# perrysou/SoftGNSS-python

Measured on NVIDIA B200. Metric: tracking channel-ms/s, higher is better.
Workload: dtype int8 x Q38 fixed-point correlators (exact int32 dot products), f64 rotors / accumulation / loop filters

## Files before the change

### softgnss_python_b200/csrc/sgx_common.cuh

```cuda
#pragma once
#include <stdint.h>
#include <stdio.h>
#include <string.h>
#include <mutex>

#ifdef SGX_EMUL
#include "cuda_emul.h"
#else
#include <cuda_runtime.h>
#define SGX_LAUNCH(kernel, grid, block, smem, stream, ...) \
  kernel<<<(grid), (block), (smem), (stream)>>>(__VA_ARGS__)
#define SGX_DYN_SMEM(name) extern __shared__ __align__(1024) unsigned char name[]
#endif

#include "../../include/softgnss_b200.h"

#ifdef SGX_EMUL
#define SGX_TABLE static
#else
#define SGX_TABLE static __constant__
#endif

namespace sgx {

// ... 87 lines not shown
#ifndef SGX_EMUL
  asm volatile("cp.async.wait_all;\n" ::: "memory");
#endif
}

__device__ __forceinline__ void mbar_init(unsigned long long* bar, unsigned count) {
#ifdef SGX_EMUL
  *bar = 0;
  (void)count;
#else
  unsigned s = (unsigned)__cvta_generic_to_shared(bar);
  asm volatile("mbarrier.init.shared::cta.b64 [%0], %1;\n" ::"r"(s), "r"(count) : "memory");
  asm volatile("fence.mbarrier_init.release.cluster;\n" ::: "memory");
#endif
}
__device__ __forceinline__ unsigned smem_addr(const void* p) {
#ifdef SGX_EMUL
  (void)p; return 0u;
#else
  unsigned a = (unsigned)__cvta_generic_to_shared(p), o;
  asm volatile("mov.u32 %0, %1;" : "=r"(o) : "r"(a));
  return o;
#endif
}
__device__ __forceinline__ unsigned lds_u32(const void* base, unsigned base_s, int byte_off) {
#ifdef SGX_EMUL
  (void)base_s; return *reinterpret_cast<const unsigned*>(reinterpret_cast<const char*>(base) + byte_off);
#else
  (void)base; unsigned v;
  asm volatile("ld.shared.u32 %0, [%1];" : "=r"(v) : "r"(base_s + (unsigned)byte_off));
  return v;
#endif
}
__device__ __forceinline__ double2 lds_f64x2(const void* base, unsigned base_s, int byte_off) {
#ifdef SGX_EMUL
  (void)base_s; return *reinterpret_cast<const double2*>(reinterpret_cast<const char*>(base) + byte_off);
#else
  (void)base; double2 v;
  asm volatile("ld.shared.v2.f64 {%0, %1}, [%2];" : "=d"(v.x), "=d"(v.y) : "r"(base_s + (unsigned)byte_off));
  return v;
#endif
}

__device__ __forceinline__ void bulk_load(void* smem_dst, const void* gsrc, unsigned bytes,
                                          unsigned long long* bar) {
#ifdef SGX_EMUL
  memcpy(smem_dst, gsrc, bytes);
  *bar += 1;
#else
  unsigned d = (unsigned)__cvta_generic_to_shared(smem_dst);
  unsigned b = (unsigned)__cvta_generic_to_shared(bar);
  asm volatile("mbarrier.arrive.expect_tx.shared::cta.b64 _, [%0], %1;\n" ::"r"(b), "r"(bytes) : "memory");
  asm volatile(
      "cp.async.bulk.shared::cluster.global.mbarrier::complete_tx::bytes [%0], [%1], %2, [%3];\n" ::"r"(d),
      "l"(gsrc), "r"(bytes), "r"(b)
      : "memory");
#endif
}
__device__ __forceinline__ void mbar_wait(unsigned long long* bar, unsigned parity) {
#ifdef SGX_EMUL
  while ((*(volatile unsigned long long*)bar & 1ull) == (unsigned long long)parity) sgx_emul::yield_to_sched();
#else
  unsigned b = (unsigned)__cvta_generic_to_shared(bar);
  asm volatile(
      "{\n"
      ".reg .pred p;\n"
// ... 25 lines not shown
```

### softgnss_python_b200/csrc/sgx_track.cu

```cuda
#include <vector>
#include <fcntl.h>
#include <sys/stat.h>
#include <unistd.h>
#include "sgx_common.cuh"

namespace sgx {

constexpr int TRK_THREADS = 256;
constexpr int TRK_WARPS = TRK_THREADS / 32;
constexpr int TRK_MARGIN = 256;

struct TrackArgs {
  const int8_t* rec;
  long long rec_stride;
  const long long* rec_len;
  const sgx_channel* ch;
  const int8_t* chips;
  double* out;
  int* ms_done;
  int* status;
  int n_channels;
  int ms;
  int resume;
  long long avail;
  struct TrackState* state;
  long long* prof;
  int win;
  long long skip;
  long long abs_base;
  double fs, codeFreqBasis, codeLength, spc;
  double c1code, c2code, c1carr, c2carr;
};

struct MsParams {
  double startE, stepE, startL, stepL, startP, stepP;
  double inv_step;
  long long q0_fix, h_fix;
  double cps;
  double rem_cyc;
  double w;
  double rem_rad;
  double fs;
  long long pos;
// ... 43 lines not shown

__device__ __forceinline__ void cis_cycles(double cyc, float& c, float& s) {
  cyc -= rint(cyc);
  const float hi = (float)cyc;
  const float lo = (float)(cyc - (double)hi) * 6.2831853071795865f;
  float s0, c0;
  sincospif(2.0f * hi, &s0, &c0);
  c = fmaf(-s0, lo, c0);
  s = fmaf(c0, lo, s0);
}

__device__ __forceinline__ void cmul(float& r, float& i, float ar, float ai, float br, float bi) {
  r = fmaf(ar, br, -(ai * bi));
  i = fmaf(ar, bi, ai * br);
}

struct CodeState {
  double codeFreq, remCodePhase, oldCodeNco, oldCodeError, nextRemCode;
  long long pos;
};
struct CarrState {
  double carrFreq, carrFreqBasis, remCarrPhase, oldCarrNco, oldCarrError, w;
};

constexpr int SGX_PAUSED = 1;

struct TrackState {
  CodeState c;
  CarrState r;
  int k;
  int status;
};

__device__ void prepare_code(const TrackArgs& a, CodeState& st, long long rec_len, MsParams& p) {
  double step = st.codeFreq / a.fs;
  int blk = (int)ceil((a.codeLength - st.remCodePhase) / step);
  p.blk = blk;
  p.pos = st.pos;
  p.stop = 0;
  long long aligned = st.pos & ~15LL;
  if (st.pos + blk > rec_len) { p.stop = SGX_ERR_SHORT; return; }
  if (st.pos + blk > a.avail) { p.stop = SGX_PAUSED; return; }
  if (blk <= 0 || (st.pos - aligned) + blk > a.win) { p.stop = SGX_ERR_RANGE; return; }
  double rem = st.remCodePhase, spc = a.spc, bs = (double)blk * step;
  p.startE = rem - spc;
  p.stepE = (((bs + rem) - spc) - p.startE) / (double)blk;
  p.startL = rem + spc;
  p.stepL = (((bs + rem) + spc) - p.startL) / (double)blk;
  p.startP = rem;
  p.stepP = ((bs + rem) - p.startP) / (double)blk;
  p.inv_step = 1.0 / step;
  p.h_fix = __double2ll_rn(0.5 * p.inv_step * 1099511627776.0);
  p.q0_fix = __double2ll_rn(-rem * p.inv_step * 1099511627776.0);
  st.nextRemCode = (lin_y(blk - 1, p.stepP, p.startP) + step) - 1023.0;
}

__device__ void prepare_carr(const TrackArgs& a, CarrState& st, MsParams& p) {
  st.w = st.carrFreq * 2.0 * 3.141592653589793;
  p.cps = (st.w / a.fs) * 0.15915494309189535;
  p.rem_cyc = st.remCarrPhase * 0.15915494309189535;
  p.w = st.w;
  p.rem_rad = st.remCarrPhase;
  p.fs = a.fs;
}

__device__ double carry_carr_phase(const TrackArgs& a, const CarrState& st, int blk) {
  const double TWO_PI = 6.283185307179586;
  double arg_end = st.w * ((double)blk / a.fs) + st.remCarrPhase;
  double m;
  if (arg_end >= 0.0) {
    double q = floor(arg_end * 0.15915494309189535);
    m = __fma_rn(-q, TWO_PI, arg_end);
    if (m < 0.0) { q -= 1.0; m = __fma_rn(-q, TWO_PI, arg_end); }
    else if (m >= TWO_PI) { q += 1.0; m = __fma_rn(-q, TWO_PI, arg_end); }
  } else {
    m = fmod(arg_end, TWO_PI);
    if (m != 0.0 && m < 0.0) m += TWO_PI;
  }
  return m;
}

__device__ __forceinline__ void correlate_groups(const MsParams& P, const int8_t* cur, const float* codeS, int tid,
                                                 double& tEr, double& tEi, double& tPr, double& tPi, double& tLr,
                                                 double& tLi) {
    const int off = (int)(P.pos - (P.pos & ~15LL));
    const int ng = (off + P.blk + 15) >> 4;
    const int gpt = (ng + TRK_THREADS - 1) / TRK_THREADS;
    const int g0 = tid * gpt;
    const int g1 = min(g0 + gpt, ng);
    if (g0 < g1) {
      int ib = 16 * g0 - off;
      const int i0 = max(ib, 0);
      CodeVar E, Pm, L;
      E.init(i0, P.startE, P.stepE, P.inv_step, codeS);
      Pm.init(i0, P.startP, P.stepP, P.inv_step, codeS);
      L.init(i0, P.startL, P.stepL, P.inv_step, codeS);
      float wr[16], wi[16], w16r, w16i, rotr, roti;
      {
        cis_cycles((double)ib * P.cps + P.rem_cyc, rotr, roti);
        float s1, c1;
        cis_cycles(P.cps, c1, s1);
// ... 233 lines not shown
  const double r2 = r * r;
  double ps = -7.647163731819816e-13;
  ps = fma(ps, r2, 1.6059043836821613e-10);
  ps = fma(ps, r2, -2.505210838544172e-08);
  ps = fma(ps, r2, 2.7557319223985893e-06);
  ps = fma(ps, r2, -1.984126984126984e-04);
  ps = fma(ps, r2, 8.333333333333333e-03);
  ps = fma(ps, r2, -1.6666666666666666e-01);
  const double s0 = fma(ps * r2, r, r);
  double pc = 4.779477332387385e-14;
  pc = fma(pc, r2, -1.1470745597729725e-11);
  pc = fma(pc, r2, 2.08767569878681e-09);
  pc = fma(pc, r2, -2.755731922398589e-07);
  pc = fma(pc, r2, 2.48015873015873e-05);
  pc = fma(pc, r2, -1.388888888888889e-03);
  pc = fma(pc, r2, 4.1666666666666664e-02);
  pc = fma(pc, r2, -0.5);
  const double c0 = fma(pc, r2, 1.0);
  const int q = (int)(long long)k & 3;
  const double sa = (q & 1) ? c0 : s0, ca = (q & 1) ? s0 : c0;
  sn = (q & 2) ? -sa : sa;
  cs = ((q + 1) & 2) ? -ca : ca;
}

__device__ __forceinline__ void cis_cycles_f64(double cyc, double& c, double& s) {
  cyc -= rint(cyc);
  sincospi(2.0 * cyc, &s, &c);
}

template <int NW>
__device__ __forceinline__ void build_exact_tables(ExactTables& T, double cps, int lane) {
  constexpr int LMAX = 4 * NW;
  constexpr int ND = ExactDigits<NW>::value;
  if (lane < LMAX) {
    double c, s;
    cis_cycles_f64((double)lane * cps, c, s);
    const double one = (double)(1LL << (8 * ND - 2));
    long long w[2] = {__double2ll_rn(c * one), __double2ll_rn(s * one)};
#pragma unroll
    for (int q = 0; q < 2; ++q) {
      long long v = w[q];
#pragma unroll
      for (int d = 0; d < ND - 1; ++d) {
        const long long b = ((v + 128) & 0xFF) - 128;
        T.tw[q][d][lane] = (signed char)b;
        v = (v - b) >> 8;
      }
      T.tw[q][ND - 1][lane] = (signed char)v;
    }
  }
  constexpr int Z0 = (LMAX + 5 <= 32) ? LMAX : 0;
  if (lane >= Z0 && lane < Z0 + 5) {
    const int j = lane - Z0;
    cis_cycles_f64((double)(LMAX - 4 + j) * cps, T.z[j][0], T.z[j][1]);
  }
}

constexpr int IRREGULAR = 1 << 30;
__device__ __noinline__ int settle_boundary(int n, const MsParams& P) {
  if ((n & 1) == 0) return max(0, min(next_event(n >> 1, P.startP, P.stepP, P.inv_step), P.blk));
  const int c = (n - 1) >> 1;
  const int b = next_event(c, P.startE, P.stepE, P.inv_step);
  const int bl = next_event(c + 1, P.startL, P.stepL, P.inv_step);
  return max(0, min(b, P.blk)) | (bl != b ? IRREGULAR : 0);
}

__device__ __noinline__ double2 start_rotor(int a, const MsParams& P) {
  const double th = P.w * ((double)a / P.fs) + P.rem_rad;
  double sn, cs;
  if (fabs(th) < 5.0e5) sincos_reduced(th, sn, cs);
  else sincos(th, &sn, &cs);
  return make_double2(cs, sn);
}

__device__ __noinline__ void correlate_per_sample(const MsParams& P, const int8_t* cur, const unsigned char* codeB, int off,
                                                  int i0, int i1, double* acc) {
  for (int i = i0; i < i1; ++i) {
    const int ie = (int)ceil(lin_y(i, P.stepE, P.startE));
    const int ip = (int)ceil(lin_y(i, P.stepP, P.startP));
    const int il = (int)ceil(lin_y(i, P.stepL, P.startL));
    double cs, sn;
    cis_cycles_f64((double)i * P.cps + P.rem_cyc, cs, sn);
    const double x = (double)cur[off + i];
    const double pr = x * cs, pi = x * sn;
    const double ce = codeB[ie] ? -1.0 : 1.0, cp = codeB[ip] ? -1.0 : 1.0, cl = codeB[il] ? -1.0 : 1.0;
    acc[0] += ce * pr; acc[1] += ce * pi;
    acc[2] += cp * pr; acc[3] += cp * pi;
    acc[4] += cl * pr; acc[5] += cl * pi;
// ... 2 lines not shown

__device__ __forceinline__ double flip_sign(double x, unsigned m) {
  return __hiloint2double(__double2hiint(x) ^ (int)m, __double2loint(x));
}

__device__ __forceinline__ double digits_to_double(int lo, int mid, int hi) {
  long long v = (long long)mid * 65536 + (long long)lo;
  v += (long long)hi << 32;
  v += 0x4338000000000000LL;
  return __longlong_as_double(v) - 6755399441055744.0;
}

template <int NW, int SEGS>
__device__ __forceinline__ void correlate_exact(const MsParams& P, const MsParams& Pcold, const int8_t* cur,
                                                const unsigned char* codeB, const ExactTables& T, int tid,
                                                double& tEr, double& tEi, double& tPr, double& tPi, double& tLr,
                                                double& tLi) {
  constexpr int LMAX = 4 * NW;
  constexpr int ND = ExactDigits<NW>::value;
  static_assert(SEGS == 8, "sign bytes are fetched for 8 half-chip segments per thread");
  const int off = (int)(P.pos - (P.pos & ~15LL));
  const int n0 = SEGS * tid - 1;
  const long long FR_ONE = 1LL << 40, FR_EPS = 1099512;
  long long qf = P.q0_fix + (long long)n0 * P.h_fix;
  auto boundary = [&](int n, long long q) -> int {
    if (n < 0) return 0;
    if (n > 2046) return P.blk;
    const long long fr = q & (FR_ONE - 1);
    if (fr < FR_EPS || fr > FR_ONE - FR_EPS) return settle_boundary(n, Pcold);
    return max(0, min((int)(q >> 40) + 1, P.blk));
  };
  int a = boundary(n0, qf);
  if ((a & ~IRREGULAR) >= P.blk) return;
  int twr[ND][NW], twi[ND][NW];
#pragma unroll
  for (int d = 0; d < ND; ++d)
#pragma unroll
    for (int q = 0; q < NW; ++q) {
      twr[d][q] = reinterpret_cast<const int*>(T.tw[0][d])[q];
      twi[d][q] = reinterpret_cast<const int*>(T.tw[1][d])[q];
    }
  unsigned sg_lo = reinterpret_cast<const unsigned*>(codeB)[tid];
  unsigned sg_hi = reinterpret_cast<const unsigned*>(codeB)[tid + 1];
  double rotr = 1.0, roti = 0.0;
  double aEr = 0, aEi = 0, aPr = 0, aPi = 0, aLr = 0, aLi = 0;
  bool fresh = true;
  const unsigned cur_s = smem_addr(cur), z_s = smem_addr(&T.z[0][0]);
#pragma unroll 1
  for (int s = 0; s < SEGS; ++s) {
    qf += P.h_fix;
    const int b = boundary(n0 + s + 1, qf);
    const int len = (b & ~IRREGULAR) - (a & ~IRREGULAR);
    if (len > 0) {
      if (len > LMAX || ((a | b) & IRREGULAR)) {
        double acc[6] = {0, 0, 0, 0, 0, 0};
        correlate_per_sample(Pcold, cur, codeB, off, a & ~IRREGULAR, b & ~IRREGULAR, acc);
        const double up = (double)(1LL << (8 * ND - 2));
        aEr += acc[0] * up; aEi += acc[1] * up; aPr += acc[2] * up; aPi += acc[3] * up; aLr += acc[4] * up; aLi += acc[5] * up;
        fresh = true;
      } else {
        const unsigned mE = sg_lo << 24, mL = __byte_perm(sg_lo, 0u, 0x1444), mP = (s & 1) ? mL : mE;
        if (fresh) {
          const double2 r0 = start_rotor(a, Pcold);
          rotr = r0.x; roti = r0.y;
          fresh = false;
        }
        const int sh = ((off + a) & 3) * 8;
        unsigned raw[NW + 1];
        {
          const int wo = (off + a) & ~3;
#pragma unroll
          for (int q = 0; q <= NW; ++q) raw[q] = lds_u32(cur, cur_s, wo + 4 * q);
        }
        unsigned w[NW];
#pragma unroll
        for (int q = 0; q < NW; ++q) w[q] = __funnelshift_r(raw[q], raw[q + 1], sh);
        w[NW - 1] &= __funnelshift_lc(0xFFFFFFFFu, 0u, max(8 * (len - 4 * (NW - 1)), 0));
        if (len < LMAX - 4) {
#pragma unroll
          for (int q = 0; q < NW - 1; ++q) w[q] &= __funnelshift_lc(0xFFFFFFFFu, 0u, max(8 * (len - 4 * q), 0));
        }
        int xr[ND], xi[ND];
#pragma unroll
        for (int d = 0; d < ND; ++d) { xr[d] = 0; xi[d] = 0; }
#pragma unroll
        for (int q = 0; q < NW; ++q) {
#pragma unroll
          for (int d = 0; d < ND; ++d) {
            xr[d] = __dp4a((int)w[q], twr[d][q], xr[d]);
            xi[d] = __dp4a((int)w[q], twi[d][q], xi[d]);
          }
        }
        const double Sr = digits_to_double(xr[1] * 256 + xr[0], xr[3] * 256 + xr[2], ND == 5 ? xr[ND - 1] : 0);
        const double Si = digits_to_double(xi[1] * 256 + xi[0], xi[3] * 256 + xi[2], ND == 5 ? xi[ND - 1] : 0);
        const double Rr = fma(rotr, Sr, -(roti * Si)), Ri = fma(rotr, Si, roti * Sr);
        aEr += flip_sign(Rr, mE); aEi += flip_sign(Ri, mE);
        aPr += flip_sign(Rr, mP); aPi += flip_sign(Ri, mP);
        aLr += flip_sign(Rr, mL); aLi += flip_sign(Ri, mL);
        const int j = len - (LMAX - 4);
        if (j >= 0) {
          const double2 z = lds_f64x2(&T.z[0][0], z_s, 16 * j);
          const double zr = z.x, zi = z.y;
          const double nr = fma(rotr, zr, -(roti * zi)), ni = fma(rotr, zi, roti * zr);
          rotr = nr; roti = ni;
        } else {
          fresh = true;
        }
      }
    }
    a = b;
    if (s & 1) { sg_lo = __funnelshift_r(sg_lo, sg_hi, 8); sg_hi >>= 8; }
  }
  const double sc = 1.0 / (double)(1LL << (8 * ND - 2));
  tEr += aEr * sc; tEi += aEi * sc; tPr += aPr * sc; tPi += aPi * sc; tLr += aLr * sc; tLi += aLi * sc;
}

template <bool BULK, int NW, bool EXACT, int NT>
__global__ void __launch_bounds__(NT, 2) track_kernel(TrackArgs a) {
  SGX_DYN_SMEM(smem);
  int8_t* buf0 = (int8_t*)smem;
  int8_t* buf1 = buf0 + a.win;
  __shared__ MsParams prm;
  constexpr int NWARPS = NT / 32;
  __shared__ double red[NWARPS][6];
  __shared__ float codeS[1040];
  __shared__ unsigned long long mbar[2];
  __shared__ ExactTables xt;
  __shared__ CodeState cstS;
  __shared__ CarrState rstS;
  __shared__ __align__(4) unsigned char codeB[EXACT ? 1040 : 4];

  const int tid = threadIdx.x;
  const int cid = blockIdx.x;
  const int rid = cid / a.n_channels;
  const sgx_channel chn = a.ch[cid];
  if (chn.prn == 0) {
    if (tid == 0) {
      a.ms_done[cid] = 0;
      a.status[cid] = SGX_OK;
      if (a.state) { a.state[cid].k = 0; a.state[cid].status = SGX_OK; }
    }
    return;
  }
  const int8_t* rec = a.rec + (long long)rid * a.rec_stride;
  const long long rec_len = a.rec_len[rid];
  const long long rec_alloc = (rec_len + 15) & ~15LL;
  {
    const int8_t* c = a.chips + (chn.prn - 1) * 1023;
    for (int i = tid; i < 1040; i += NT) {
      codeS[i] = i < 1025 ? (float)c[(i + 1022) % 1023] : 0.f;
      if (EXACT) codeB[i] = codeS[i] < 0.f ? 0x80 : 0;
    }
  }
  int k_start = 0;
  if (a.resume) {
    const TrackState* ts = a.state + cid;
    if (ts->status != SGX_PAUSED) return;
    k_start = ts->k;
    if (tid == 0) { CodeState c = ts->c; prepare_code(a, c, rec_len, prm); cstS = c; }
    if (tid == 32) { CarrState r = ts->r; prepare_carr(a, r, prm); rstS = r; }
    if (tid == 0 && BULK) { mbar_init(&mbar[0], 1); mbar_init(&mbar[1], 1); }
  } else {
    if (tid == 0) {
      CodeState c;
      c.codeFreq = a.codeFreqBasis;
      c.remCodePhase = 0.0;
      c.oldCodeNco = c.oldCodeError = 0.0;
      c.nextRemCode = 0.0;
      c.pos = a.skip + (long long)chn.codePhase;
      prepare_code(a, c, rec_len, prm);
      cstS = c;
      if (BULK) { mbar_init(&mbar[0], 1); mbar_init(&mbar[1], 1); }
    }
    if (tid == 32) {
      CarrState r;
      r.carrFreq = chn.acquiredFreq;
      r.carrFreqBasis = chn.acquiredFreq;
      r.remCarrPhase = 0.0;
      r.oldCarrNco = r.oldCarrError = 0.0;
      prepare_carr(a, r, prm);
      rstS = r;
    }
  }
  if (EXACT && (tid >> 5) == 1) {
    const double cps = __shfl_sync(0xffffffffu, tid == 32 ? prm.cps : 0.0, 0);
    build_exact_tables<(NW > 0 ? NW : 1)>(xt, cps, tid & 31);
  }
  __syncthreads();

  auto stage = [&](int8_t* dst, long long pos) {
    long long al = pos & ~15LL;
    long long nb = rec_alloc - al;
    if (nb > a.win) nb = a.win;
    if (nb <= 0) return 0;
    if (BULK) {
      return (int)nb;
    } else {
      const int8_t* src = rec + al;
      for (int o = tid * 16; o < (int)nb; o += NT * 16) cp_async16(dst + o, src + o);
      cp_async_commit();
      return (int)nb;
    }
  };
  unsigned phase0 = 0, phase1 = 0;
  bool pending0 = false, pending1 = false;
  if (prm.stop == 0) {
    const int par = k_start & 1;
    int nb = stage(par ? buf1 : buf0, prm.pos);
    if (BULK) {
      if (nb > 0) {
        if (tid == 0) bulk_load(par ? buf1 : buf0, rec + (prm.pos & ~15LL), (unsigned)nb, &mbar[par]);
        if (par) pending1 = true; else pending0 = true;
      }
    }
  }

  int k = k_start;
  for (; k < a.ms; ++k) {
    const MsParams P = prm;
    if (P.stop != 0) break;
    long long t0 = 0, t1 = 0, t2 = 0, t3 = 0;
    if (a.prof && (tid == 0 || tid == 64)) t0 = clock64();
    int8_t* cur = (k & 1) ? buf1 : buf0;
    int8_t* nxt = (k & 1) ? buf0 : buf1;
    if (BULK) {
      if (k & 1) { if (pending1) { mbar_wait(&mbar[1], phase1); phase1 ^= 1; pending1 = false; } }
      else       { if (pending0) { mbar_wait(&mbar[0], phase0); phase0 ^= 1; pending0 = false; } }
    } else {
      if (k == k_start) { cp_async_wait_all(); __syncthreads(); }
    }
    {
      long long npos = P.pos + P.blk;
      int nb = stage(nxt, npos);
      if (BULK && nb > 0) {
        if (tid == 0) bulk_load(nxt, rec + (npos & ~15LL), (unsigned)nb, &mbar[(k + 1) & 1]);
        if (k & 1) pending0 = true; else pending1 = true;
      }
    }

    double tEr = 0.0, tEi = 0.0, tPr = 0.0, tPi = 0.0, tLr = 0.0, tLi = 0.0;
    if (EXACT)       correlate_exact<(NW > 0 ? NW : 1), 2048 / NT>(P, prm, cur, codeB, xt, tid, tEr, tEi, tPr, tPi, tLr, tLi);
    else if (NW > 0) correlate_segments<(NW > 0 ? NW : 1)>(P, cur, codeS, tid, tEr, tEi, tPr, tPi, tLr, tLi);
    else             correlate_groups(P, cur, codeS, tid, tEr, tEi, tPr, tPi, tLr, tLi);
    if (a.prof && (tid == 0 || tid == 64)) t1 = clock64();
    double v0 = warp_sum_f64(tEi), v1 = warp_sum_f64(tEr), v2 = warp_sum_f64(tPi), v3 = warp_sum_f64(tPr),
           v4 = warp_sum_f64(tLi), v5 = warp_sum_f64(tLr);
    if ((tid & 31) == 0) {
      double* r = red[tid >> 5];
      r[0] = v0; r[1] = v1; r[2] = v2; r[3] = v3; r[4] = v4; r[5] = v5;
    }
    if (!BULK) cp_async_wait_all();
    __syncthreads();
    if (a.prof && (tid == 0 || tid == 64)) t2 = clock64();
    if (tid == 0) {
      CodeState cst = cstS;
      double I_E = 0.0, Q_E = 0.0, I_L = 0.0, Q_L = 0.0;
      for (int w = 0; w < NWARPS; ++w) { I_E += red[w][0]; Q_E += red[w][1]; I_L += red[w][4]; Q_L += red[w][5]; }
      cst.remCodePhase = cst.nextRemCode;
      cst.pos = P.pos + P.blk;
      double em = sqrt(I_E * I_E + Q_E * Q_E), lm = sqrt(I_L * I_L + Q_L * Q_L);
      double codeError = (em - lm) / (em + lm);
      double codeNco = cst.oldCodeNco + a.c1code * (codeError - cst.oldCodeError) + codeError * a.c2code;
      cst.oldCodeNco = codeNco;
      cst.oldCodeError = codeError;
      cst.codeFreq = a.codeFreqBasis - codeNco;
      if (k + 1 < a.ms) prepare_code(a, cst, rec_len, prm);
      double* o = a.out + (long long)cid * SGX_TRACK_FIELDS * a.ms + k;
      const long long m = a.ms;
      o[0 * m] = (double)(cst.pos + a.abs_base);
      o[1 * m] = cst.codeFreq;
      o[4 * m] = I_E; o[5 * m] = I_L; o[6 * m] = Q_E; o[8 * m] = Q_L;
      o[9 * m] = codeError; o[10 * m] = codeNco;
      cstS = cst;
    } else if (tid == 32) {
      CarrState rst = rstS;
      double I_P = 0.0, Q_P = 0.0;
      for (int w = 0; w < NWARPS; ++w) { I_P += red[w][2]; Q_P += red[w][3]; }
      rst.remCarrPhase = carry_carr_phase(a, rst, P.blk);
      double carrError = atan(Q_P / I_P) * 0.5 / 3.141592653589793;
      double carrNco = rst.oldCarrNco + a.c1carr * (carrError - rst.oldCarrError) + carrError * a.c2carr;
      rst.oldCarrNco = carrNco;
      rst.oldCarrError = carrError;
      rst.carrFreq = rst.carrFreqBasis + carrNco;
      if (k + 1 < a.ms) prepare_carr(a, rst, prm);
      double* o = a.out + (long long)cid * SGX_TRACK_FIELDS * a.ms + k;
      const long long m = a.ms;
      o[2 * m] = rst.carrFreq;
      o[3 * m] = I_P; o[7 * m] = Q_P;
      o[11 * m] = carrError; o[12 * m] = carrNco;
      rstS = rst;
    }
    if (EXACT && (tid >> 5) == 1 && k + 1 < a.ms) {
      const double cps = __shfl_sync(0xffffffffu, tid == 32 ? prm.cps : 0.0, 0);
      build_exact_tables<(NW > 0 ? NW : 1)>(xt, cps, tid & 31);
    }
    if (a.prof && tid == 0) t3 = clock64();
    __syncthreads();
    if (a.prof && (tid == 0 || tid == 64)) {
      const long long t4 = clock64();
      long long* pr = a.prof + (long long)cid * 8 + (tid == 0 ? 0 : 4);
      pr[0] += t1 - t0; pr[1] += t2 - t1; pr[2] += (tid == 0 ? t3 - t2 : 0); pr[3] += t4 - (tid == 0 ? t3 : t2);
    }
  }
  if (BULK) {
    if (pending0) mbar_wait(&mbar[0], phase0);
    if (pending1) mbar_wait(&mbar[1], phase1);
  } else {
    cp_async_wait_all();
  }
  if (tid == 0) {
    const int status = (k == a.ms) ? SGX_OK : prm.stop;
    a.ms_done[cid] = k;
    a.status[cid] = status;
    if (a.state) { a.state[cid].c = cstS; a.state[cid].k = k; a.state[cid].status = status; }
  }
  if (tid == 32 && a.state) a.state[cid].r = rstS;
}

struct TrackScratch {
  DevBuf rec, len, ch, chips, out, done, status, state, prof;
  cudaStream_t copy_stream = nullptr;
  cudaEvent_t ev[2] = {nullptr, nullptr};
  int8_t* pin[2] = {nullptr, nullptr};
  size_t pin_cap = 0;
  cudaEvent_t pin_ev[2] = {nullptr, nullptr};
};

struct FileSrc {
  int fd;
  int sample_bytes;
  long long base;
  long long len;
  long long chunk;
  int bad_value;
};
static TrackScratch g_trk;

static bool use_bulk() {
  const char* e = getenv("SGX_TRK_STAGE");
  return !(e && strcmp(e, "cpasync") == 0);
}

}

using namespace sgx;

static int track_core(const int8_t* rec, int64_t rec_stride, const int64_t* rec_len,
                      int32_t n_recordings, const sgx_channel* ch, int32_t n_channels,
                      const sgx_settings* st, const int8_t* ca_chips, double* out,
// ... 20 lines not shown
  } else if (((rec_stride & 15) && n_recordings > 1) || ((uintptr_t)rec & 15)) {
    return fail(SGX_ERR_ARG, "sgx_track", "device recordings must be 16-byte aligned with a stride multiple of 16");
  }
  if (g_trk.len.reserve(sizeof(long long) * n_recordings) || g_trk.ch.reserve(sizeof(sgx_channel) * nch) ||
      g_trk.chips.reserve(32 * 1023) || g_trk.done.reserve(sizeof(int) * nch) ||
      g_trk.status.reserve(sizeof(int) * nch) || g_trk.state.reserve(sizeof(TrackState) * nch))
    return fail(SGX_ERR_CUDA, "cudaMalloc", "tracking scratch");
  SGX_CUDA(cudaMemcpyAsync(g_trk.len.p, rec_len, sizeof(long long) * n_recordings, cudaMemcpyHostToDevice, s));
  SGX_CUDA(cudaMemcpyAsync(g_trk.ch.p, ch, sizeof(sgx_channel) * nch, cudaMemcpyHostToDevice, s));
  SGX_CUDA(cudaMemcpyAsync(g_trk.chips.p, ca_chips, 32 * 1023, cudaMemcpyHostToDevice, s));
  const size_t out_bytes = sizeof(double) * (size_t)nch * SGX_TRACK_FIELDS * ms;
  double* d_out = out;
  const bool out_on_host = !is_device_ptr(out);
  if (out_on_host) {
    if (g_trk.out.reserve(out_bytes)) return fail(SGX_ERR_CUDA, "cudaMalloc", "tracking output");
    d_out = g_trk.out.as<double>();
  }

  TrackArgs a;
  a.rec = d_rec;
  a.rec_stride = stride;
  a.rec_len = g_trk.len.as<long long>();
  a.ch = g_trk.ch.as<sgx_channel>();
  a.chips = g_trk.chips.as<int8_t>();
  a.out = d_out;
  a.ms_done = g_trk.done.as<int>();
  a.status = g_trk.status.as<int>();
  a.n_channels = n_channels;
  a.ms = ms;
  a.resume = 0;
  a.avail = 0x7fffffffffffffffLL;
  a.state = g_trk.state.as<TrackState>();
  a.prof = nullptr;
  if (getenv("SGX_TRK_PROF")) {
    if (g_trk.prof.reserve(sizeof(long long) * 8 * nch)) return fail(SGX_ERR_CUDA, "cudaMalloc", "prof");
    SGX_CUDA(cudaMemsetAsync(g_trk.prof.p, 0, sizeof(long long) * 8 * nch, s));
    a.prof = g_trk.prof.as<long long>();
  }
  a.win = win;
  a.skip = file ? st->skipNumberOfBytes / file->sample_bytes - file->base : st->skipNumberOfBytes;
  a.abs_base = file ? file->base : 0;
  a.fs = st->samplingFreq;
  a.codeFreqBasis = st->codeFreqBasis;
  a.codeLength = (double)st->codeLength;
  a.spc = st->dllCorrelatorSpacing;
  a.c1code = st->tau2code / st->tau1code;
  a.c2code = st->PDIcode / st->tau1code;
  a.c1carr = st->tau2carr / st->tau1carr;
  a.c2carr = st->PDIcarr / st->tau1carr;

  const size_t smem = 2 * (size_t)win;
  auto launch = [&]() -> int {
  const double half_chip = st->samplingFreq / (2.0 * st->codeFreqBasis);
  int nw = ((int)ceil(half_chip + 0.25) + 3) / 4;
  bool exact = true;
  if (const char* e = getenv("SGX_TRK_KERNEL")) {
    if (strcmp(e, "groups") == 0) nw = 0;
    if (strcmp(e, "segments") == 0) exact = false;
  }
  if (fabs(st->dllCorrelatorSpacing - 0.5) > 1e-12) nw = 0;
  const bool bulk = use_bulk();
#define SGX_TRK_GO_NT(B, W, X, NTHR)                                                               \
  {                                                                                                \
    auto kfn = track_kernel<B, W, X, NTHR>;                                                        \
    SGX_CUDA(cudaFuncSetAttribute(kfn, cudaFuncAttributeMaxDynamicSharedMemorySize, (int)smem));   \
    SGX_COUNTED_LAUNCH(kfn, dim3(nch), dim3(NTHR), smem, s, a);                                    \
  }
#define SGX_TRK_GO(B, W, X) SGX_TRK_GO_NT(B, W, X, TRK_THREADS)
#define SGX_TRK_EXACT(W) { if (bulk) SGX_TRK_GO(true, W, true) else SGX_TRK_GO(false, W, true) }
// ... 46 lines not shown
          if (r <= 0) return fail(SGX_ERR_ARG, "sgx_track_file", "short read from the recording file");
          got += (size_t)r;
        }
        if (file->sample_bytes == 2) {
          const int16_t* src = (const int16_t*)hb;
          for (long long i = 0; i < width; ++i) {
            const int v = src[i];
            if (v < -128 || v > 127) file->bad_value = 1;
            hb[i] = (int8_t)v;
          }
          if (file->bad_value) return fail(SGX_ERR_ARG, "sgx_track_file", "int16 sample outside the int8 range of the correlators");
        }
        SGX_CUDA(cudaMemcpyAsync(g_trk.rec.as<int8_t>() + off, hb, (size_t)width, cudaMemcpyHostToDevice, g_trk.copy_stream));
        SGX_CUDA(cudaEventRecord(g_trk.pin_ev[c & 1], g_trk.copy_stream));
      } else
      SGX_CUDA(cudaMemcpy2DAsync(g_trk.rec.as<int8_t>() + off, (size_t)stride, rec + off, (size_t)rec_stride, (size_t)width,
                                 (size_t)n_recordings, cudaMemcpyHostToDevice, g_trk.copy_stream));
      SGX_CUDA(cudaEventRecord(g_trk.ev[0], g_trk.copy_stream));
      SGX_CUDA(cudaStreamWaitEvent(s, g_trk.ev[0], 0));
      a.avail = off + width;
      a.resume = c > 0;
      int rc0 = launch();
      if (rc0) return rc0;
    }
  }
  SGX_CUDA(cudaGetLastError());
  if (out_on_host) SGX_CUDA(cudaMemcpyAsync(out, d_out, out_bytes, cudaMemcpyDeviceToHost, s));
  std::vector<int> h_status_v(nch);
  int* h_status = h_status_v.data();
  SGX_CUDA(cudaMemcpyAsync(ms_done, a.ms_done, sizeof(int) * nch, cudaMemcpyDeviceToHost, s));
  SGX_CUDA(cudaMemcpyAsync(h_status, a.status, sizeof(int) * nch, cudaMemcpyDeviceToHost, s));
  SGX_CUDA(cudaStreamSynchronize(s));
  if (a.prof) {
    long long* hp = (long long*)malloc(sizeof(long long) * 8 * nch);
    cudaMemcpy(hp, a.prof, sizeof(long long) * 8 * nch, cudaMemcpyDeviceToHost);
    double acc[8] = {0, 0, 0, 0, 0, 0, 0, 0};
    for (int i = 0; i < nch; ++i) for (int j = 0; j < 8; ++j) acc[j] += (double)hp[i * 8 + j];
    const double per = (double)nch * ms;
    fprintf(stderr, "[sgx prof] cycles/period thread0: correlate %.0f reduce+bar %.0f bookkeeping %.0f bar %.0f | thread64: correlate %.0f reduce+bar %.0f wait-for-bookkeeping %.0f\n",
            acc[0] / per, acc[1] / per, acc[2] / per, acc[3] / per, acc[4] / per, acc[5] / per, acc[7] / per);
    free(hp);
  }
  int rc = SGX_OK;
  for (int i = 0; i < nch; ++i)
    if (h_status[i] != SGX_OK && rc == SGX_OK) rc = h_status[i];
  if (rc == SGX_ERR_SHORT) return fail(rc, "sgx_track", "Not able to read the specified number of samples for tracking");
  if (rc != SGX_OK) return fail(rc, "sgx_track", "loop state left the supported range");
  return SGX_OK;
}

extern "C" int sgx_track(const int8_t* rec, int64_t rec_stride, const int64_t* rec_len,
                         int32_t n_recordings, const sgx_channel* ch, int32_t n_channels,
                         const sgx_settings* st, const int8_t* ca_chips, double* out,
                         int32_t* ms_done, void* cuda_stream) {
  if (sgx_device_count() <= 0) return fail(SGX_ERR_NODEV, "sgx_track", "no CUDA device");
  SGX_API_GUARD();
  return track_core(rec, rec_stride, rec_len, n_recordings, ch, n_channels, st, ca_chips, out, ms_done, cuda_stream,
                    nullptr);
}

extern "C" int sgx_track_file(const char* path, int32_t sample_bytes, const sgx_channel* ch, int32_t n_channels,
                              const sgx_settings* st, const int8_t* ca_chips, double* out, int32_t* ms_done,
                              int64_t chunk_samples, int64_t* window ,
                              void* cuda_stream) {
  if (sgx_device_count() <= 0) return fail(SGX_ERR_NODEV, "sgx_track_file", "no CUDA device");
  SGX_API_GUARD();
  if (!path || !ch || !st || n_channels <= 0 || (sample_bytes != 1 && sample_bytes != 2))
    return fail(SGX_ERR_ARG, "sgx_track_file", "null pointer, or dataType other than int8 / int16");
  const int fd = open(path, O_RDONLY);
  if (fd < 0) return fail(SGX_ERR_ARG, "sgx_track_file", "cannot open the recording file");
  struct stat sb;
  if (fstat(fd, &sb) != 0) { close(fd); return fail(SGX_ERR_ARG, "sgx_track_file", "cannot stat the recording file"); }
  const long long file_samples = (long long)sb.st_size / sample_bytes;
  double cp_min = 1e300, cp_max = -1e300;
// ... 36 lines not shown
```

Baseline: 34.88 million.

## Shorten serial per-ms bookkeeping and issue next bulk prefetch earlier

The single-thread code and carrier loop-filter bookkeeping becomes warp-wide, with divisions and square roots split across lanes through shuffles. The carrier phase carry moves to warp 2 so it runs before correlation, and the exact twiddle table build now happens inside the carrier warp. The bulk load for the next-next millisecond is issued from bookkeeping right after prepare_code, which deepens prefetch to two buffers ahead. Correlator sample loads now use 128-bit shared loads plus a lane shuffle, and a leading empty segment is skipped. The per-warp profiling is also reworked. These changes aim to cut the serial critical path between __syncthreads, but they add shuffle overhead and more complex buffer and barrier parity handling.

```diff
diff --git a/softgnss_python_b200/csrc/sgx_common.cuh b/softgnss_python_b200/csrc/sgx_common.cuh
--- a/softgnss_python_b200/csrc/sgx_common.cuh
+++ b/softgnss_python_b200/csrc/sgx_common.cuh
@@ -143,6 +143,16 @@
   return v;
 #endif
 }
+__device__ __forceinline__ uint4 lds_u32x4(const void* base, unsigned base_s, int byte_off) {
+#ifdef SGX_EMUL
+  (void)base_s; return *reinterpret_cast<const uint4*>(reinterpret_cast<const char*>(base) + byte_off);
+#else
+  (void)base; uint4 v;
+  asm volatile("ld.shared.v4.u32 {%0, %1, %2, %3}, [%4];" : "=r"(v.x), "=r"(v.y), "=r"(v.z), "=r"(v.w)
+               : "r"(base_s + (unsigned)byte_off));
+  return v;
+#endif
+}
 __device__ __forceinline__ double2 lds_f64x2(const void* base, unsigned base_s, int byte_off) {
 #ifdef SGX_EMUL
   (void)base_s; return *reinterpret_cast<const double2*>(reinterpret_cast<const char*>(base) + byte_off);
diff --git a/softgnss_python_b200/csrc/sgx_track.cu b/softgnss_python_b200/csrc/sgx_track.cu
--- a/softgnss_python_b200/csrc/sgx_track.cu
+++ b/softgnss_python_b200/csrc/sgx_track.cu
@@ -9,6 +9,7 @@
 constexpr int TRK_THREADS = 256;
 constexpr int TRK_WARPS = TRK_THREADS / 32;
 constexpr int TRK_MARGIN = 256;
+constexpr int TRK_PROF_N = 5;
 
 struct TrackArgs {
   const int8_t* rec;
@@ -118,41 +119,54 @@
   int status;
 };
 
-__device__ void prepare_code(const TrackArgs& a, CodeState& st, long long rec_len, MsParams& p) {
-  double step = st.codeFreq / a.fs;
-  int blk = (int)ceil((a.codeLength - st.remCodePhase) / step);
-  p.blk = blk;
-  p.pos = st.pos;
-  p.stop = 0;
-  long long aligned = st.pos & ~15LL;
-  if (st.pos + blk > rec_len) { p.stop = SGX_ERR_SHORT; return; }
-  if (st.pos + blk > a.avail) { p.stop = SGX_PAUSED; return; }
-  if (blk <= 0 || (st.pos - aligned) + blk > a.win) { p.stop = SGX_ERR_RANGE; return; }
-  double rem = st.remCodePhase, spc = a.spc, bs = (double)blk * step;
-  p.startE = rem - spc;
-  p.stepE = (((bs + rem) - spc) - p.startE) / (double)blk;
-  p.startL = rem + spc;
-  p.stepL = (((bs + rem) + spc) - p.startL) / (double)blk;
-  p.startP = rem;
-  p.stepP = ((bs + rem) - p.startP) / (double)blk;
-  p.inv_step = 1.0 / step;
-  p.h_fix = __double2ll_rn(0.5 * p.inv_step * 1099511627776.0);
-  p.q0_fix = __double2ll_rn(-rem * p.inv_step * 1099511627776.0);
-  st.nextRemCode = (lin_y(blk - 1, p.stepP, p.startP) + step) - 1023.0;
-}
-
-__device__ void prepare_carr(const TrackArgs& a, CarrState& st, MsParams& p) {
+__device__ void prepare_code(const TrackArgs& a, CodeState& st, long long rec_len, MsParams& p, int lane) {
+  const double step = st.codeFreq / a.fs;
+  const double q = (lane == 1 ? 1.0 : a.codeLength - st.remCodePhase) / step;
+  const int blk = (int)ceil(__shfl_sync(0xffffffffu, q, 0));
+  const double inv_step = __shfl_sync(0xffffffffu, q, 1);
+  const long long aligned = st.pos & ~15LL;
+  int stop = 0;
+  if (st.pos + blk > rec_len) stop = SGX_ERR_SHORT;
+  else if (st.pos + blk > a.avail) stop = SGX_PAUSED;
+  else if (blk <= 0 || (st.pos - aligned) + blk > a.win) stop = SGX_ERR_RANGE;
+  if (lane == 0) { p.blk = blk; p.pos = st.pos; p.stop = stop; }
+  if (stop) return;
+  const double rem = st.remCodePhase, spc = a.spc, bs = (double)blk * step;
+  const double startE = rem - spc, startL = rem + spc, startP = rem;
+  const double num = lane == 0 ? ((bs + rem) - spc) - startE : lane == 1 ? ((bs + rem) + spc) - startL : (bs + rem) - startP;
+  const double d = num / (double)blk;
+  const double stepE = __shfl_sync(0xffffffffu, d, 0), stepL = __shfl_sync(0xffffffffu, d, 1),
+               stepP = __shfl_sync(0xffffffffu, d, 2);
+  if (lane == 0) {
+    p.startE = startE; p.stepE = stepE;
+    p.startL = startL; p.stepL = stepL;
+    p.startP = startP; p.stepP = stepP;
+    p.inv_step = inv_step;
+    p.h_fix = __double2ll_rn(0.5 * inv_step * 1099511627776.0);
+    p.q0_fix = __double2ll_rn(-rem * inv_step * 1099511627776.0);
+  }
+  st.nextRemCode = (lin_y(blk - 1, stepP, startP) + step) - 1023.0;
+}
+
+__device__ double prepare_carr(const TrackArgs& a, CarrState& st, MsParams& p, bool write) {
   st.w = st.carrFreq * 2.0 * 3.141592653589793;
-  p.cps = (st.w / a.fs) * 0.15915494309189535;
-  p.rem_cyc = st.remCarrPhase * 0.15915494309189535;
-  p.w = st.w;
-  p.rem_rad = st.remCarrPhase;
-  p.fs = a.fs;
-}
-
-__device__ double carry_carr_phase(const TrackArgs& a, const CarrState& st, int blk) {
+  const double cps = (st.w / a.fs) * 0.15915494309189535;
+  if (write) {
+    p.cps = cps;
+    p.w = st.w;
+    p.fs = a.fs;
+  }
+  return cps;
+}
+
+__device__ __forceinline__ void set_carr_phase(MsParams& p, double rem) {
+  p.rem_cyc = rem * 0.15915494309189535;
+  p.rem_rad = rem;
+}
+
+__device__ double carry_carr_phase(double w, double rem, int blk, double fs) {
   const double TWO_PI = 6.283185307179586;
-  double arg_end = st.w * ((double)blk / a.fs) + st.remCarrPhase;
+  double arg_end = w * ((double)blk / fs) + rem;
   double m;
   if (arg_end >= 0.0) {
     double q = floor(arg_end * 0.15915494309189535);
@@ -452,9 +466,16 @@
 __device__ __forceinline__ void build_exact_tables(ExactTables& T, double cps, int lane) {
   constexpr int LMAX = 4 * NW;
   constexpr int ND = ExactDigits<NW>::value;
-  if (lane < LMAX) {
+  constexpr int Z0 = (LMAX + 5 <= 32) ? LMAX : 0;
+  const bool tw = lane < LMAX, zs = lane >= Z0 && lane < Z0 + 5;
+  if (tw || (Z0 > 0 && zs)) {
     double c, s;
-    cis_cycles_f64((double)lane * cps, c, s);
+    cis_cycles_f64((double)(tw ? lane : LMAX - 4 + (lane - Z0)) * cps, c, s);
+    if (!tw) {
+      T.z[lane - Z0][0] = c;
+      T.z[lane - Z0][1] = s;
+      return;
+    }
     const double one = (double)(1LL << (8 * ND - 2));
     long long w[2] = {__double2ll_rn(c * one), __double2ll_rn(s * one)};
 #pragma unroll
@@ -469,11 +490,7 @@
       T.tw[q][ND - 1][lane] = (signed char)v;
     }
   }
-  constexpr int Z0 = (LMAX + 5 <= 32) ? LMAX : 0;
-  if (lane >= Z0 && lane < Z0 + 5) {
-    const int j = lane - Z0;
-    cis_cycles_f64((double)(LMAX - 4 + j) * cps, T.z[j][0], T.z[j][1]);
-  }
+  if (Z0 == 0 && zs) cis_cycles_f64((double)(LMAX - 4 + lane) * cps, T.z[lane][0], T.z[lane][1]);
 }
 
 constexpr int IRREGULAR = 1 << 30;
@@ -542,6 +559,11 @@
   };
   int a = boundary(n0, qf);
   if ((a & ~IRREGULAR) >= P.blk) return;
+  int s0 = 0;
+  if (n0 < 0) {
+    const int b0 = boundary(0, qf + P.h_fix);
+    if ((b0 & ~IRREGULAR) == (a & ~IRREGULAR)) { s0 = 1; qf += P.h_fix; a = b0; }
+  }
   int twr[ND][NW], twi[ND][NW];
 #pragma unroll
   for (int d = 0; d < ND; ++d)
@@ -557,7 +579,7 @@
   bool fresh = true;
   const unsigned cur_s = smem_addr(cur), z_s = smem_addr(&T.z[0][0]);
 #pragma unroll 1
-  for (int s = 0; s < SEGS; ++s) {
+  for (int s = s0; s < SEGS; ++s) {
     qf += P.h_fix;
     const int b = boundary(n0 + s + 1, qf);
     const int len = (b & ~IRREGULAR) - (a & ~IRREGULAR);
@@ -578,9 +600,20 @@
         const int sh = ((off + a) & 3) * 8;
         unsigned raw[NW + 1];
         {
-          const int wo = (off + a) & ~3;
-#pragma unroll
-          for (int q = 0; q <= NW; ++q) raw[q] = lds_u32(cur, cur_s, wo + 4 * q);
+          constexpr int NQ = (NW + 7) / 4;
+          const int ab = (off + a) & ~15, j = ((off + a) >> 2) & 3;
+          unsigned wd[4 * NQ];
+#pragma unroll
+          for (int q = 0; q < NQ; ++q) {
+            uint4 v = make_uint4(0u, 0u, 0u, 0u);
+            if (q < NQ - 1 || j + NW >= 4 * (NQ - 1)) v = lds_u32x4(cur, cur_s, ab + 16 * q);
+            wd[4 * q] = v.x; wd[4 * q + 1] = v.y; wd[4 * q + 2] = v.z; wd[4 * q + 3] = v.w;
+          }
+          unsigned t[NW + 2];
+#pragma unroll
+          for (int q = 0; q < NW + 2; ++q) t[q] = (j & 2) ? wd[q + 2] : wd[q];
+#pragma unroll
+          for (int q = 0; q <= NW; ++q) raw[q] = (j & 1) ? t[q + 1] : t[q];
         }
         unsigned w[NW];
 #pragma unroll
@@ -639,8 +672,11 @@
   __shared__ CodeState cstS;
   __shared__ CarrState rstS;
   __shared__ __align__(4) unsigned char codeB[EXACT ? 1040 : 4];
+  __shared__ long long stampS[NWARPS][TRK_PROF_N + 1];
+  __shared__ double remNextS;
 
   const int tid = threadIdx.x;
+  const int lane = tid & 31;
   const int cid = blockIdx.x;
   const int rid = cid / a.n_channels;
   const sgx_channel chn = a.ch[cid];
@@ -667,28 +703,29 @@
     const TrackState* ts = a.state + cid;
     if (ts->status != SGX_PAUSED) return;
     k_start = ts->k;
-    if (tid == 0) { CodeState c = ts->c; prepare_code(a, c, rec_len, prm); cstS = c; }
-    if (tid == 32) { CarrState r = ts->r; prepare_carr(a, r, prm); rstS = r; }
+    if (tid < 32) { CodeState c = ts->c; prepare_code(a, c, rec_len, prm, lane); if (lane == 0) cstS = c; }
+    if (tid == 32) { CarrState r = ts->r; prepare_carr(a, r, prm, true); set_carr_phase(prm, r.remCarrPhase); rstS = r; }
     if (tid == 0 && BULK) { mbar_init(&mbar[0], 1); mbar_init(&mbar[1], 1); }
   } else {
-    if (tid == 0) {
+    if (tid < 32) {
       CodeState c;
       c.codeFreq = a.codeFreqBasis;
       c.remCodePhase = 0.0;
       c.oldCodeNco = c.oldCodeError = 0.0;
       c.nextRemCode = 0.0;
       c.pos = a.skip + (long long)chn.codePhase;
-      prepare_code(a, c, rec_len, prm);
-      cstS = c;
-      if (BULK) { mbar_init(&mbar[0], 1); mbar_init(&mbar[1], 1); }
-    }
+      prepare_code(a, c, rec_len, prm, lane);
+      if (lane == 0) cstS = c;
+    }
+    if (tid == 0 && BULK) { mbar_init(&mbar[0], 1); mbar_init(&mbar[1], 1); }
     if (tid == 32) {
       CarrState r;
       r.carrFreq = chn.acquiredFreq;
       r.carrFreqBasis = chn.acquiredFreq;
       r.remCarrPhase = 0.0;
       r.oldCarrNco = r.oldCarrError = 0.0;
-      prepare_carr(a, r, prm);
+      prepare_carr(a, r, prm, true);
+      set_carr_phase(prm, r.remCarrPhase);
       rstS = r;
     }
   }
@@ -722,6 +759,9 @@
         if (tid == 0) bulk_load(par ? buf1 : buf0, rec + (prm.pos & ~15LL), (unsigned)nb, &mbar[par]);
         if (par) pending1 = true; else pending0 = true;
       }
+      const long long npos = prm.pos + prm.blk;
+      const int nb1 = stage(par ? buf0 : buf1, npos);
+      if (tid == 0 && nb1 > 0 && k_start < a.ms) bulk_load(par ? buf0 : buf1, rec + (npos & ~15LL), (unsigned)nb1, &mbar[par ^ 1]);
     }
   }
 
@@ -729,8 +769,9 @@
   for (; k < a.ms; ++k) {
     const MsParams P = prm;
     if (P.stop != 0) break;
-    long long t0 = 0, t1 = 0, t2 = 0, t3 = 0;
-    if (a.prof && (tid == 0 || tid == 64)) t0 = clock64();
+    const bool stamp = a.prof && (tid & 31) == 0;
+    long long* ts = stampS[tid >> 5];
+    if (stamp) ts[0] = clock64();
     int8_t* cur = (k & 1) ? buf1 : buf0;
     int8_t* nxt = (k & 1) ? buf0 : buf1;
     if (BULK) {
@@ -743,16 +784,17 @@
       long long npos = P.pos + P.blk;
       int nb = stage(nxt, npos);
       if (BULK && nb > 0) {
-        if (tid == 0) bulk_load(nxt, rec + (npos & ~15LL), (unsigned)nb, &mbar[(k + 1) & 1]);
         if (k & 1) pending0 = true; else pending1 = true;
       }
     }
+    if (tid == 64) remNextS = carry_carr_phase(P.w, P.rem_rad, P.blk, P.fs);
+    if (stamp) ts[1] = clock64();
 
     double tEr = 0.0, tEi = 0.0, tPr = 0.0, tPi = 0.0, tLr = 0.0, tLi = 0.0;
     if (EXACT)       correlate_exact<(NW > 0 ? NW : 1), 2048 / NT>(P, prm, cur, codeB, xt, tid, tEr, tEi, tPr, tPi, tLr, tLi);
     else if (NW > 0) correlate_segments<(NW > 0 ? NW : 1)>(P, cur, codeS, tid, tEr, tEi, tPr, tPi, tLr, tLi);
     else             correlate_groups(P, cur, codeS, tid, tEr, tEi, tPr, tPi, tLr, tLi);
-    if (a.prof && (tid == 0 || tid == 64)) t1 = clock64();
+    if (stamp) ts[2] = clock64();
     double v0 = warp_sum_f64(tEi), v1 = warp_sum_f64(tEr), v2 = warp_sum_f64(tPi), v3 = warp_sum_f64(tPr),
            v4 = warp_sum_f64(tLi), v5 = warp_sum_f64(tLr);
     if ((tid & 31) == 0) {
@@ -761,55 +803,69 @@
     }
     if (!BULK) cp_async_wait_all();
     __syncthreads();
-    if (a.prof && (tid == 0 || tid == 64)) t2 = clock64();
-    if (tid == 0) {
+    if (stamp) ts[3] = clock64();
+    if (tid < 32) {
       CodeState cst = cstS;
+      const int blk = prm.blk;
+      __syncwarp();
       double I_E = 0.0, Q_E = 0.0, I_L = 0.0, Q_L = 0.0;
       for (int w = 0; w < NWARPS; ++w) { I_E += red[w][0]; Q_E += red[w][1]; I_L += red[w][4]; Q_L += red[w][5]; }
       cst.remCodePhase = cst.nextRemCode;
-      cst.pos = P.pos + P.blk;
-      double em = sqrt(I_E * I_E + Q_E * Q_E), lm = sqrt(I_L * I_L + Q_L * Q_L);
+      cst.pos = cst.pos + blk;
+      const double mag = sqrt(lane == 1 ? I_L * I_L + Q_L * Q_L : I_E * I_E + Q_E * Q_E);
+      const double em = __shfl_sync(0xffffffffu, mag, 0), lm = __shfl_sync(0xffffffffu, mag, 1);
       double codeError = (em - lm) / (em + lm);
       double codeNco = cst.oldCodeNco + a.c1code * (codeError - cst.oldCodeError) + codeError * a.c2code;
       cst.oldCodeNco = codeNco;
       cst.oldCodeError = codeError;
       cst.codeFreq = a.codeFreqBasis - codeNco;
-      if (k + 1 < a.ms) prepare_code(a, cst, rec_len, prm);
-      double* o = a.out + (long long)cid * SGX_TRACK_FIELDS * a.ms + k;
-      const long long m = a.ms;
-      o[0 * m] = (double)(cst.pos + a.abs_base);
-      o[1 * m] = cst.codeFreq;
-      o[4 * m] = I_E; o[5 * m] = I_L; o[6 * m] = Q_E; o[8 * m] = Q_L;
-      o[9 * m] = codeError; o[10 * m] = codeNco;
-      cstS = cst;
-    } else if (tid == 32) {
+      if (k + 1 < a.ms) prepare_code(a, cst, rec_len, prm, lane);
+      if (lane == 0) {
+        cstS = cst;
+        if (BULK && k + 1 < a.ms && prm.stop == 0) {
+          const long long npos = prm.pos + prm.blk;
+          const int nb = stage(cur, npos);
+          if (nb > 0) bulk_load(cur, rec + (npos & ~15LL), (unsigned)nb, &mbar[k & 1]);
+        }
+        double* o = a.out + (long long)cid * SGX_TRACK_FIELDS * a.ms + k;
+        const long long m = a.ms;
+        o[0 * m] = (double)(cst.pos + a.abs_base);
+        o[1 * m] = cst.codeFreq;
+        o[4 * m] = I_E; o[5 * m] = I_L; o[6 * m] = Q_E; o[8 * m] = Q_L;
+        o[9 * m] = codeError; o[10 * m] = codeNco;
+      }
+    } else if (tid < 64) {
       CarrState rst = rstS;
+      __syncwarp();
       double I_P = 0.0, Q_P = 0.0;
       for (int w = 0; w < NWARPS; ++w) { I_P += red[w][2]; Q_P += red[w][3]; }
-      rst.remCarrPhase = carry_carr_phase(a, rst, P.blk);
       double carrError = atan(Q_P / I_P) * 0.5 / 3.141592653589793;
       double carrNco = rst.oldCarrNco + a.c1carr * (carrError - rst.oldCarrError) + carrError * a.c2carr;
       rst.oldCarrNco = carrNco;
       rst.oldCarrError = carrError;
       rst.carrFreq = rst.carrFreqBasis + carrNco;
-      if (k + 1 < a.ms) prepare_carr(a, rst, prm);
-      double* o = a.out + (long long)cid * SGX_TRACK_FIELDS * a.ms + k;
-      const long long m = a.ms;
-      o[2 * m] = rst.carrFreq;
-      o[3 * m] = I_P; o[7 * m] = Q_P;
-      o[11 * m] = carrError; o[12 * m] = carrNco;
-      rstS = rst;
-    }
-    if (EXACT && (tid >> 5) == 1 && k + 1 < a.ms) {
-      const double cps = __shfl_sync(0xffffffffu, tid == 32 ? prm.cps : 0.0, 0);
-      build_exact_tables<(NW > 0 ? NW : 1)>(xt, cps, tid & 31);
-    }
-    if (a.prof && tid == 0) t3 = clock64();
+      if (k + 1 < a.ms) {
+        const double cps = prepare_carr(a, rst, prm, lane == 0);
+        if (EXACT) build_exact_tables<(NW > 0 ? NW : 1)>(xt, cps, lane);
+      }
+      if (lane == 0) {
+        double* o = a.out + (long long)cid * SGX_TRACK_FIELDS * a.ms + k;
+        const long long m = a.ms;
+        o[2 * m] = rst.carrFreq;
+        o[3 * m] = I_P; o[7 * m] = Q_P;
+        o[11 * m] = carrError; o[12 * m] = carrNco;
+        rstS = rst;
+      }
+    } else if (tid == 64) {
+      set_carr_phase(prm, remNextS);
+    }
+    if (stamp) ts[4] = clock64();
     __syncthreads();
-    if (a.prof && (tid == 0 || tid == 64)) {
-      const long long t4 = clock64();
-      long long* pr = a.prof + (long long)cid * 8 + (tid == 0 ? 0 : 4);
-      pr[0] += t1 - t0; pr[1] += t2 - t1; pr[2] += (tid == 0 ? t3 - t2 : 0); pr[3] += t4 - (tid == 0 ? t3 : t2);
+    if (stamp) {
+      ts[5] = clock64();
+      long long* pr = a.prof + ((long long)cid * NWARPS + (tid >> 5)) * TRK_PROF_N;
+#pragma unroll
+      for (int i = 0; i < TRK_PROF_N; ++i) pr[i] += ts[i + 1] - ts[i];
     }
   }
   if (BULK) {
@@ -824,7 +880,11 @@
     a.status[cid] = status;
     if (a.state) { a.state[cid].c = cstS; a.state[cid].k = k; a.state[cid].status = status; }
   }
-  if (tid == 32 && a.state) a.state[cid].r = rstS;
+  if (tid == 32 && a.state) {
+    CarrState r = rstS;
+    r.remCarrPhase = prm.rem_rad;
+    a.state[cid].r = r;
+  }
 }
 
 struct TrackScratch {
@@ -911,9 +971,10 @@
   a.avail = 0x7fffffffffffffffLL;
   a.state = g_trk.state.as<TrackState>();
   a.prof = nullptr;
+  const size_t prof_n = (size_t)nch * TRK_WARPS * TRK_PROF_N;
   if (getenv("SGX_TRK_PROF")) {
-    if (g_trk.prof.reserve(sizeof(long long) * 8 * nch)) return fail(SGX_ERR_CUDA, "cudaMalloc", "prof");
-    SGX_CUDA(cudaMemsetAsync(g_trk.prof.p, 0, sizeof(long long) * 8 * nch, s));
+    if (g_trk.prof.reserve(sizeof(long long) * prof_n)) return fail(SGX_ERR_CUDA, "cudaMalloc", "prof");
+    SGX_CUDA(cudaMemsetAsync(g_trk.prof.p, 0, sizeof(long long) * prof_n, s));
     a.prof = g_trk.prof.as<long long>();
   }
   a.win = win;
@@ -1026,14 +1087,18 @@
   SGX_CUDA(cudaMemcpyAsync(h_status, a.status, sizeof(int) * nch, cudaMemcpyDeviceToHost, s));
   SGX_CUDA(cudaStreamSynchronize(s));
   if (a.prof) {
-    long long* hp = (long long*)malloc(sizeof(long long) * 8 * nch);
-    cudaMemcpy(hp, a.prof, sizeof(long long) * 8 * nch, cudaMemcpyDeviceToHost);
-    double acc[8] = {0, 0, 0, 0, 0, 0, 0, 0};
-    for (int i = 0; i < nch; ++i) for (int j = 0; j < 8; ++j) acc[j] += (double)hp[i * 8 + j];
+    std::vector<long long> hp(prof_n);
+    cudaMemcpy(hp.data(), a.prof, sizeof(long long) * prof_n, cudaMemcpyDeviceToHost);
     const double per = (double)nch * ms;
-    fprintf(stderr, "[sgx prof] cycles/period thread0: correlate %.0f reduce+bar %.0f bookkeeping %.0f bar %.0f | thread64: correlate %.0f reduce+bar %.0f wait-for-bookkeeping %.0f\n",
-            acc[0] / per, acc[1] / per, acc[2] / per, acc[3] / per, acc[4] / per, acc[5] / per, acc[7] / per);
-    free(hp);
+    fprintf(stderr, "[sgx prof] cycles/period  warp:  wait+prefetch  correlate  reduce+bar  bookkeeping  bar  | period\n");
+    for (int w = 0; w < TRK_WARPS; ++w) {
+      double acc[TRK_PROF_N] = {}, tot = 0.0;
+      for (int i = 0; i < nch; ++i)
+        for (int j = 0; j < TRK_PROF_N; ++j) acc[j] += (double)hp[((size_t)i * TRK_WARPS + w) * TRK_PROF_N + j];
+      for (int j = 0; j < TRK_PROF_N; ++j) tot += acc[j];
+      fprintf(stderr, "[sgx prof] %d: %8.0f %8.0f %8.0f %8.0f %8.0f | %8.0f\n", w, acc[0] / per, acc[1] / per, acc[2] / per,
+              acc[3] / per, acc[4] / per, tot / per);
+    }
   }
   int rc = SGX_OK;
   for (int i = 0; i < nch; ++i)
```

New measurement: 37.09 million, median of 6. 6.3% higher.
